# RemoteSensingTools/vSmartMOM.jl

Hardware: AMD Instinct MI355X
Metric: spectral-points/s (whole node) for rt_run, O2-A band (higher is better)
Workload: dtype f64; 1 GPU; C2: O2-A 759-770 nm, nStokes=3, Nquad=20 (N=60), 40 layers, 10000 spectral points/GPU, m=0..2, Rayleigh+synthetic O2 absorption, Lambertian 0.15; ranks=1, collective_backend=none (1 rank), N=60, layers=40, points_per_gpu=10000, fourier_moments=3

## Files before the change

include/vsmartmom_hip.h:

```cpp
#ifndef VSMARTMOM_HIP_H
#define VSMARTMOM_HIP_H

#include <stddef.h>
#include <stdint.h>

#ifdef __cplusplus
extern "C" {
#endif

typedef enum vsm_status {
  VSM_OK = 0,
  VSM_ERR_INVALID_ARG = 1,
  VSM_ERR_UNSUPPORTED = 2,
  VSM_ERR_HIP = 3,
  VSM_ERR_NO_DEVICE = 4
} vsm_status;

typedef enum vsm_iface {
  VSM_IFACE_00 = 0,
  VSM_IFACE_01 = 1,
  VSM_IFACE_10 = 2,
  VSM_IFACE_11 = 3
} vsm_iface;

// ... 387 lines not shown
int vsm_run_create_view_f64(const vsm_quad_f64* q, int S, int nm, const int* m_h, const int* coupling_h, void* workspace,
                            size_t workspace_bytes, unsigned flags, int nrows, const int* rows_h, vsm_run** run);
int vsm_run_create_view_f32(const vsm_quad_f32* q, int S, int nm, const int* m_h, const int* coupling_h, void* workspace,
                            size_t workspace_bytes, unsigned flags, int nrows, const int* rows_h, vsm_run** run);
int vsm_run_layer_f64(vsm_run* run, int ndoubl, const double* dtau, const double* varpi, const double* tau_sum,
                      const double* F0, int ncomp, const double* const* Zpp, const double* const* Zmp, long long z_stride,
                      const double* fcomp, int toa, const int* layer_coupling_h, void* stream);
int vsm_run_layer_f32(vsm_run* run, int ndoubl, const float* dtau, const float* varpi, const float* tau_sum,
                      const float* F0, int ncomp, const float* const* Zpp, const float* const* Zmp, long long z_stride,
                      const float* fcomp, int toa, const int* layer_coupling_h, void* stream);
int vsm_run_export_f64(vsm_run* run, const vsm_composite_f64* comps, void* stream);
int vsm_run_export_f32(vsm_run* run, const vsm_composite_f32* comps, void* stream);
int vsm_run_import_f64(vsm_run* run, const vsm_composite_f64* comps, void* stream);
int vsm_run_import_f32(vsm_run* run, const vsm_composite_f32* comps, void* stream);
int vsm_run_zw_tail(vsm_run* run);
int vsm_run_view_rows(vsm_run* run, int nrows, const int* rows_h);
int vsm_run_view_block(const vsm_run* run, int block, int* im, int* n, int* nv, int* local_rows);
int vsm_run_view_rows(vsm_run* run, int nrows, const int* rows_h);
int vsm_run_view_block(const vsm_run* run, int block, int* im, int* n, int* nv, int* local_rows);
int vsm_run_destroy(vsm_run* run);
enum { VSM_SURFACE_LAMBERTIAN_SCALAR = 0, VSM_SURFACE_LAMBERTIAN_SPECTRAL = 1, VSM_SURFACE_BRDF = 2 };
enum { VSM_SURFACE_LAYER_IDENTITY = 1 };
unsigned vsm_surface_layer_flags(int kind, int m, int has_surface_source);
int vsm_run_export_moment_f64(vsm_run* run, int im, const vsm_composite_f64* comp, void* stream);
int vsm_run_export_moment_f32(vsm_run* run, int im, const vsm_composite_f32* comp, void* stream);
int vsm_run_export_sources_f64(vsm_run* run, int im, const vsm_composite_f64* comp, void* stream);
int vsm_run_export_sources_f32(vsm_run* run, int im, const vsm_composite_f32* comp, void* stream);
int vsm_run_surface_f64(vsm_run* run, int im, int iface, const vsm_added_f64* added_surface, int identity, int matrices,
                        const vsm_composite_f64* comp, double* work, void* stream);
int vsm_run_surface_f32(vsm_run* run, int im, int iface, const vsm_added_f32* added_surface, int identity, int matrices,
                        const vsm_composite_f32* comp, float* work, void* stream);
int vsm_run_guard_once(vsm_run* run);
int vsm_run_counters(const vsm_run* run, int* counts_h);
int vsm_stokes_coupling_f64(int N, int n_stokes, int nblocks, const double* Zpp, const double* Zmp, int* mask_d, void* stream);
int vsm_stokes_coupling_f32(int N, int n_stokes, int nblocks, const float* Zpp, const float* Zmp, int* mask_d, void* stream);

typedef struct vsm_added_rs_f64 {
  double *ier_mp, *iet_pp, *ier_pm, *iet_mm;
  double *ieJ0_p, *ieJ0_m;
  int K;
  int reserved;
} vsm_added_rs_f64;
typedef struct vsm_added_rs_f32 {
  float *ier_mp, *iet_pp, *ier_pm, *iet_mm;
  float *ieJ0_p, *ieJ0_m;
  int K;
  int reserved;
} vsm_added_rs_f32;
typedef struct vsm_composite_rs_f64 {
  double *ieR_mp, *ieR_pm, *ieT_pp, *ieT_mm;
  double *ieJ0_p, *ieJ0_m;
  int K;
  int reserved;
} vsm_composite_rs_f64;
typedef struct vsm_composite_rs_f32 {
  float *ieR_mp, *ieR_pm, *ieT_pp, *ieT_mm;
  float *ieJ0_p, *ieJ0_m;
  int K;
  int reserved;
} vsm_composite_rs_f32;
typedef struct vsm_rrs_f64 {
  const int* shift;
  const double* varpi_ie;
  const double* fscatt;
  const double* Zpp;
  const double* Zmp;
// ... 306 lines not shown
```

vsmartmom.jl_amd/_lib.py:

```python
from __future__ import annotations

import ctypes as C
import os

_HERE = os.path.dirname(os.path.abspath(__file__))
LIB_PATH = os.environ.get("VSM_LIB_PATH") or os.path.join(_HERE, "lib", "libvsmartmom_hip.so")


class VSMError(RuntimeError):
    pass


class vsm_quad_f64(C.Structure):
    _fields_ = [("mu", C.c_void_p), ("wt", C.c_void_p), ("N", C.c_int), ("n_stokes", C.c_int),
                ("i_mu0", C.c_int), ("mu0", C.c_double)]


class vsm_quad_f32(C.Structure):
    _fields_ = [("mu", C.c_void_p), ("wt", C.c_void_p), ("N", C.c_int), ("n_stokes", C.c_int),
                ("i_mu0", C.c_int), ("mu0", C.c_float)]


class vsm_added(C.Structure):
    _fields_ = [("r_mp", C.c_void_p), ("t_pp", C.c_void_p), ("r_pm", C.c_void_p), ("t_mm", C.c_void_p),
# ... 115 lines not shown
    "vsm_interaction_inelastic_rrs_{T}": (_I, [_I, _I, _I, _P, _P, _P, _P, _P, _P, _P]),
    "vsm_copy_added_to_composite_ie_{T}": (_I, [_I, _I, _P, _P, _P]),
    "vsm_postprocess_vza_ie_{T}": (_I, [_I, _I, _I, _I, _I, _P, _P, _P, _P, _P, _P, _P]),
    "vsm_ss_column_{T}": (_I, [_P, _I, _I, _I, _P, _P, _P, _P, _P, _P, _P, _P, _P, _P, _I, _P, _P, _P, _P, _P, _P, _P]),
    "vsm_ss_column_lin_{T}": (_I, [_P, _I, _I, _I, _I, _I, _I, _I, _I, _P, _P, _P, _P, _P, _P, _P, _P, _P, _P, _I, _P, _P, _P, _P, _P, _P, _P,
                                   _P, _P, _I, _P, _P, _P, _P, _P]),
    "vsm_ss_column_rrs_{T}": (_I, [_P, _I, _I, _I, _I, _P, _P, _P, _P, _P, _P, _P, _P, _I, _I, _P, _P, _P, _P, _P]),
    "vsm_ss_column_rrs_lin_{T}": (_I, [_P, _I, _I, _I, _I, _I, _I, _I, _I, _P, _P, _P, _P, _P, _P, _P, _P, _P, _P, _P, _I, _I, _P, _P, _P,
                                       _P, _P]),
    "vsm_exact_ss_path1_{T}": (_I, [_I, _I, _I, _I, _I, _P, _P, _P, _P, "{R}", _P, _P, _P]),
    "vsm_exact_ss_path2_{T}": (_I, [_I, _I, _I, _I, _I, _P, _P, _I, _P, "{R}", _P, _P, _P]),
    "vsm_exact_ss_path34_{T}": (_I, [_I, _I, _I, _I, _I, _P, _P, _P, _P, _P, _P, _P, _P, "{R}", _P, _P, _P, _P]),
    "vsm_exact_ss_jac12_{T}": (_I, [_I, _I, _I, _I, _I, _P, _P, _P, _P, _I, _P, "{R}", _P, _P, _P, _P, _P, _P, _P]),
    "vsm_run_supported": (_I, [_I, _I, _I]),
    "vsm_run_workspace_bytes": (_SZ, [_I, _I, _I, _I, _P]),
    "vsm_run_supported_f32": (_I, [_I, _I, _I]),
    "vsm_run_workspace_bytes_f32": (_SZ, [_I, _I, _I, _I, _P]),
    "vsm_run_create_{T}": (_I, [_P, _I, _I, _P, _P, _P, _SZ, _P]),
    "vsm_run_create_ex_{T}": (_I, [_P, _I, _I, _P, _P, _P, _SZ, C.c_uint, _P]),
    "vsm_run_create_view_{T}": (_I, [_P, _I, _I, _P, _P, _P, _SZ, C.c_uint, _I, _P, _P]),
    "vsm_run_layer_{T}": (_I, [_P, _I, _P, _P, _P, _P, _I, _P, _P, _LL, _P, _I, _P, _P]),
    "vsm_run_export_{T}": (_I, [_P, _P, _P]),
    "vsm_run_import_{T}": (_I, [_P, _P, _P]),
    "vsm_run_zw_tail": (_I, [_P]),
    "vsm_run_view_rows": (_I, [_P, _I, _P]),
    "vsm_run_view_block": (_I, [_P, _I, _P, _P, _P, _P]),
    "vsm_run_destroy": (_I, [_P]),
    "vsm_surface_layer_flags": (C.c_uint, [_I, _I, _I]),
    "vsm_run_export_moment_{T}": (_I, [_P, _I, _P, _P]),
    "vsm_run_export_sources_{T}": (_I, [_P, _I, _P, _P]),
    "vsm_run_surface_{T}": (_I, [_P, _I, _I, _P, _I, _I, _P, _P, _P]),
    "vsm_run_guard_once": (_I, [_P]),
    "vsm_run_counters": (_I, [_P, _P]),
    "vsm_stokes_coupling_{T}": (_I, [_I, _I, _I, _P, _P, _P, _P]),
    "vsm_level_radiance_work_elems": (_SZ, [_I, _I]),
    "vsm_level_radiance_{T}": (_I, [_I, _I, _I, _I, _P, _P, _P, _P, _P, _LL, _P, _P, _P, _P, _P, _P, _P]),
    "vsm_level_radiance_oplevel_{T}": (_I, [_I, _I, _I, _I, _P, _P, _P, _P, _P, _LL, _P, _P, _P, _P, _P, _P, _P]),
    "vsm_level_radiance_src_{T}": (_I, [_I, _I, _I, _I, _P, _P, _P, _I, _P, _P, _LL, _P, _P, _P, _P, _P, _P, _P]),
    "vsm_level_flux_{T}": (_I, [_I, _I, _I, _P, _I, _P, _P, _LL, _P, _I, _P, _P, "{R}", _P, _P, _P, _P]),
    "vsm_surface_emission_response_{T}": (_I, [_I, _I, _I, _I, _P, _I, _P, _P, _P, _P, _P, _LL, _P, _P, _P]),
    "vsm_level_radiance_ie_{T}": (_I, [_I, _I, _I, _I, _P, _I, _P, _P, _P, _P, _LL, _P, _P, _P, _P, _P, _P, _P, _P, _P, _P, _P]),
    "vsm_level_flux_ie_{T}": (_I, [_I, _I, _I, _I, _P, _P, _P, _LL, _P, _P, _P, _P, _P, _P, _I, _P, _P, "{R}", _P, _P, _P, _P]),
    "vsm_level_radiance_lin_{T}": (_I, [_I, _I, _I, _I, _I, _I, _P, _P, _P, _P, _LL, _P, _P, _P, _LL, _P, _P, _LL, _LL, _P, _P, _P, _P, _P,
                                        _P]),
    "vsm_level_radiance_lin_src_{T}": (_I, [_I, _I, _I, _I, _I, _I, _I, _P, _P, _P, _P, _LL, _P, _P, _P, _LL, _P, _P, _LL, _LL, _P, _P, _P,
                                            _P, _P, _P, _P, _P]),
    "vsm_level_flux_lin_{T}": (_I, [_I, _I, _I, _I, _I, _I, _P, _P, _LL, _P, _P, _P, _LL, _P, _P, _LL, _LL, _P, _P, _P, _I, _P, _P,
                                    "{R}", _P, _P, _P, _I, _P, _P]),
    "vsm_mie_work_elems": (_SZ, [_I, _I, _I]),
    "vsm_mie_nai2": (_I, [_I, _I, _I, C.c_double, C.c_double, C.c_double, _P, _P, _P, _P, _P, _P, _P, _P, _P, _P, _P]),
    "vsm_mie_lin_work_elems": (_SZ, [_I, _I, _I]),
    "vsm_mie_nai2_lin": (_I, [_I, _I, _I, C.c_double, C.c_double, C.c_double] + [_P] * 16),
    "vsm_dbge_work_elems": (_SZ, [_I, _I]),
    "vsm_truncate_dbge": (_I, [_I, _I, _I, C.c_double, _P, _P, _P, _P, _P, _P, _P, _P, _P, _P]),
    "vsm_dbge_lin_work_elems": (_SZ, [_I, _I]),
    "vsm_truncate_dbge_lin": (_I, [_I, _I, _I, C.c_double] + [_P] * 15),
    "vsm_absorption_chunk": (_I, []),
    "vsm_absorption_work_elems": (_SZ, [_I, _I]),
    "vsm_absorption_xsec": (_I, [_I, _I, _I, _I] + [_P] * 15 + [C.c_double, C.c_double, _I, _I, _I, _P, _P, _P]),
    "vsm_absorption_lin_chunk": (_I, []),
    "vsm_absorption_lin_work_elems": (_SZ, [_I, _I]),
    "vsm_absorption_xsec_lin": (_I, [_I, _I, _I, _I] + [_P] * 16 + [C.c_double, C.c_double, _I, _I, _I] + [_P] * 6),
    "vsm_absorption_profile_slots": (_I, [_I, _I, _I] + [_P] * 6),
    "vsm_absorption_lut_chunk": (_I, []),
    "vsm_absorption_lut_span": (_I, []),
    "vsm_absorption_lut_work_elems": (_SZ, [_I, _I, _I, _I]),
# ... 107 lines not shown
```

vsmartmom.jl_amd/core_rt.py:

```python
from __future__ import annotations

import contextlib
import ctypes as C
import dataclasses
import math
import os
import warnings
from dataclasses import dataclass
from typing import List, Optional

import numpy as np
import torch

from . import _lib
from . import host_model as H
from .architectures import GPU, CPU, architecture, array_type, devi, synchronize_if_gpu, to_host

IFACE = {"00": 0, "01": 1, "10": 2, "11": 3}
MOMENT_BATCH = 4
MOMENT_BATCH_MAX = 24
MOMENT_BATCHING = True
THERMAL_FUSION = True
NATIVE_RUN = True
NATIVE_SOURCES_ONLY = True
NATIVE_VIEW_ROWS = True
VIEW_ROWS_MAX = 16
NATIVE_ZW_TAIL = True
NATIVE_IDENTITY_SURFACE = True
NATIVE_DROPIN = True
REFERENCE_ORDER = False


def _require_gpu(arch):
    if not isinstance(arch, GPU):
        raise _lib.VSMError("vsmartmom.jl_amd provides the MI355X path only; architecture %r has no compute path here "
                            "(no CPU fallback by design)" % (arch,))
    if not torch.cuda.is_available():
        raise _lib.VSMError("no MI355X visible to HIP (torch.cuda.is_available() is False)")
    if arch.device_index != torch.cuda.current_device():
        raise _lib.VSMError("architecture GPU(%d) is not the current HIP device (%d): one process per GPU -- call "
                            "torch.cuda.set_device(%d) first" % (arch.device_index, torch.cuda.current_device(),
                                                                 arch.device_index))


def _torch_dtype(FT):
    return torch.float64 if np.dtype(FT) == np.float64 else torch.float32


def _stream_ptr():
    return C.c_void_p(torch.cuda.current_stream().cuda_stream)


def _ptr(t: Optional[torch.Tensor]):
    return C.c_void_p(0 if t is None else t.data_ptr())


def to_device_matrix(A: np.ndarray, arch, FT) -> torch.Tensor:
    A = np.asarray(A, dtype=FT)
    if A.ndim == 2:
        A = A[None]
    return array_type(arch)(np.ascontiguousarray(A.transpose(0, 2, 1)))
# ... 1020 lines not shown
                               work=self.work, keep_added=keep_added)
            if iz + 1 in tops_at:
                for k, comp in zip(rest, comps_l):
                    keep_top(k, iz + 1, comp.snapshot_top())

    def _native_moments(self):
        if not NATIVE_RUN or getattr(self, "coupling", None) is None or not self.moments:
            return set()
        eps2 = 2 * np.finfo(self.FT).eps
        for iz, ly in enumerate(self.moments[0]["layers"]):
            p = ly["props"]
            if p.max_tau_varpi <= eps2 or (iz > 0 and ly["iface"] != "11") or (p.fcomp is not None and p.fcomp.shape[1] > 4):
                return set()
        return {i for i, mom in enumerate(self.moments) if run_supported(self.dt, self.N, self.pol.n, int(self.coupling[mom["m"]]))}

    def _run_layers_native(self, group, comps, sources_only: bool = True, export_at=None, view_rows=None, keep_native: bool = False):
        L = _lib.lib()
        self._drop_lazy()
        nm, N, S, ns = len(group), self.N, self.S, self.pol.n
        marr = (C.c_int * nm)(*[int(mom["m"]) for mom in group])
        carr = (C.c_int * nm)(*[int(self.coupling[mom["m"]]) for mom in group])
        nbytes = run_workspace_bytes(self.dt, N, ns, S, nm, carr)
        ws = getattr(self, "_native_ws", None)
        if ws is None or ws.numel() * 8 < nbytes:
            ws = self._native_ws = _lib.poison(torch.empty(max(nbytes // 8, 2), dtype=torch.float64, device=self.dev))
        q = self.dq.cstruct()
        run = C.c_void_p()
        run_create_(self.dt, q, S, nm, marr, carr, ws, nbytes, sources_only, view_rows, run)
        ref = RunRef(run, self.__dict__.setdefault("_run_counts", {}), keep=(ws, self.dq))
        try:
            _lib.check(L.vsm_run_guard_once(run))
            if NATIVE_ZW_TAIL and not torch.cuda.is_current_stream_capturing():
                _lib.check(L.vsm_run_zw_tail(run))
            for iz in range(self.Nz):
                ly0 = group[0]["layers"][iz]
                props = [mom["layers"][iz]["props"] for mom in group]
                p0 = props[0]
                zpp = (C.c_void_p * nm)(*[p.Zpp.data_ptr() for p in props])
                zmp = (C.c_void_p * nm)(*[p.Zmp.data_ptr() for p in props])
                ncomp = 0 if p0.fcomp is None else int(p0.fcomp.shape[1])
                lc = (C.c_int * nm)(*[self._layer_coupling(mom["m"], iz) for mom in group])
                run_layer_native_(run, nm, int(ly0["nd"]), ly0["dtau"], p0.varpi, ly0["tau_sum"], self.F0, ncomp, zpp, zmp,
                                  0 if ncomp else p0.z_stride, p0.fcomp, iz == 0, lc, self.dt)
                if export_at and (iz + 1) in export_at:
                    cc = (type(comps[0].cstruct()) * nm)(*[c.cstruct() for c in comps])
                    _lib.call("vsm_run_export", self.dt, run, cc, _stream_ptr())
                    export_at[iz + 1](comps)
            if keep_native:
                for im, (mom, c) in enumerate(zip(group, comps)):
                    c.drop_native()
                    mask = int(self.coupling[mom["m"]])
                    c._native = NativeSlot(run, int(mom["m"]), mask, stokes_groups(ns, mask), ref, im)
                    ref.refs += 1
            else:
                cc = (type(comps[0].cstruct()) * nm)(*[c.cstruct() for c in comps])
                _lib.call("vsm_run_export", self.dt, run, cc, _stream_ptr())
        finally:
            ref.release()

    def thermal_slot(self) -> "ThermalSlot":
        if self._thermal is None:
            self._thermal = ThermalSlot(self)
        return self._thermal

    def _thermal_slot(self, mom, weight):
        th = self.thermal_slot()
# ... 175 lines not shown
```

vsmartmom.jl_amd/csrc/vsm_elemental.h:

```cpp
#pragma once
#include "vsm_common.h"

namespace vsm {

template <typename T>
__device__ __forceinline__ T expm1_small(T y) {
  T q = T(1.0 / 39916800.0);
  q = fma(q, y, T(1.0 / 3628800.0));
  q = fma(q, y, T(1.0 / 362880.0));
  q = fma(q, y, T(1.0 / 40320.0));
  q = fma(q, y, T(1.0 / 5040.0));
  q = fma(q, y, T(1.0 / 720.0));
  q = fma(q, y, T(1.0 / 120.0));
  q = fma(q, y, T(1.0 / 24.0));
  q = fma(q, y, T(1.0 / 6.0));
  q = fma(q, y, T(0.5));
  q = fma(q, y, T(1.0));
  return q * y;
}
template <typename T>
__device__ __forceinline__ T expdiff_tab_thin(T xi, T xj, T ai, T aj, T ej) {
  const T dlt = xi - xj;
  return (fabs(dlt) > T(0.125) * fmax(xi, xj)) ? (ai - aj) : ej * expm1_small<T>(-dlt);
}
template <typename T>
__device__ __forceinline__ T expdiff_tab_thick(T xi, T xj, T ei, T ej) {
  const T dlt = xi - xj;
  const T v = ((dlt < T(0)) ? ei : ej) * (-expm1(-fabs(dlt)));
  return (dlt < T(0)) ? v : -v;
}

__device__ __forceinline__ double geo_div(double a, double b) { return a / b; }
__device__ __forceinline__ float geo_div(float a, float b) { return __fdividef(a, b); }

template <typename T>
__device__ __forceinline__ void elemental_pair(T w, T zp, T zm, T mi, T xi, T ai, T ei, T mj, T xj, T aj, T ej, T wct, bool diag,
                                               bool thick, T& rr, T& tt) {
  rr = w * zm * geo_div(mj, mi + mj) * wct * (-(ai + aj + ai * aj));
  T ediff;
  if (thick) ediff = expdiff_tab_thick<T>(xi, xj, ei, ej); else ediff = expdiff_tab_thin<T>(xi, xj, ai, aj, ej);
  const T t_off = w * zp * geo_div(mj, mi - mj) * wct * ediff;
  const T t_1 = w * zp * xi * wct;
  const T t_same = diag ? ei * (T(1) + t_1) : ej * t_1;
  tt = (mi == mj) ? t_same : t_off;
}

}
```

vsmartmom.jl_amd/csrc/vsm_native.hip:

```cpp
#include <stdlib.h>

#include <vector>

#include "vsm_native_dev.h"
#include "vsm_native_run.h"

#ifndef VSM_NATIVE_PARK_RT
#define VSM_NATIVE_PARK_RT 3
#endif

namespace vsm {

struct nlayer_comps {
  double* c[NSUB_MAX];
};

namespace {

template <int RT, int KS, int KZ = KS, bool TILE = false>
__device__ __forceinline__ void ned_body(nsmem<RT, (4 * KS + 2 > 16 * RT)>& sm, npos<RT>& p, int n, int gsz, unsigned uvmask, int ndoubl,
                                         const double* __restrict__ img, nstrip<RT>& r_s, nstrip<RT>& t_s, int* status) {
  using G = ngeo<RT>;
  constexpr unsigned dP = 0, dQ = G::AF * 8;
  double* jp = sm.vec[0];
// ... 1153 lines not shown
    }
    R[naf_idx<RT>(i, j)] = rv;
    T[naf_idx<RT>(i, j)] = tv;
  }
  if (ph == 0) {
    const int i0 = ns * q.i_mu0;
    const double mu0n = q.mu[i0];
    const double x0 = d / mu0n, e0 = exp(-x0), a0 = expm1(-x0);
    double zp = 0.0, zm = 0.0;
    for (int qq = 0; qq < ns; ++qq) {
      const long long zo = fi + (long long)N * (i0 + qq);
      const double f = F0[qq + (long long)ns * s];
      zp += zget(Zp, zo) * f;
      zm += zget(Zm, zo) * f;
    }
    double rr, tt;
    elemental_pair(w, zp, zm, mi, xi, ai, ei, mu0n, x0, a0, e0, (m == 0) ? 0.5 : 0.25, false, thick || x0 >= 0.5, rr, tt);
    const double att = exp(-tau_sum[s] / mu0n);
    const double vp = (i < n) ? tt * att : 0.0;
    const double vm = (i < n) ? rr * att * sg : 0.0;
    const double expk0 = exp(-d / q.mu0);
    out[2 * G::AF + i] = vp;
    out[2 * G::AF + NP + i] = vm;
    out[2 * G::AF + 2 * NP + i] = expk0;
    if (riders_in) {
      T[naf_idx<RT>(i, c1)] = vp;
      T[naf_idx<RT>(i, c2)] = vm * expk0;
      R[naf_idx<RT>(i, c1)] = vm;
      R[naf_idx<RT>(i, c2)] = vp;
    }
  }
}

template <typename T>
struct ngroup_map {
  int ngroups;
  int grp_of[4];
  int pos_in[4];
  int gsz[4];
  int rt[4];
  int n[4];
  T* base[4];
};
__device__ __forceinline__ int nat_idx_rt(const double*, int rt, int i, int j) {
  const int w = j >> 4, l15 = j & 15, ta = i >> 4, mm = i & 15, kq = mm & 3, r = mm >> 2;
  const int lane = (kq << 4) | l15, u = 2 * ta + (r >> 1);
  return ((w * 2 * rt + u) * 64 + lane) * 2 + (r & 1);
}
__device__ __forceinline__ int nat_idx_rt(const float*, int rt, int i, int j) {
  const int w = j >> 4, l15 = j & 15, ta = i >> 4, mm = i & 15, kq = mm & 3, r = mm >> 2;
  return ((w * rt + ta) * 64 + ((kq << 4) | l15)) * 4 + r;
}
__device__ __forceinline__ void nat_elem_rt(const double*, int rt, int e, int& i, int& j) {
  const int half = e & 1, lane = (e >> 1) & 63, unit = (e >> 7) % (2 * rt), w = (e >> 7) / (2 * rt);
  i = 16 * (unit >> 1) + (lane >> 4) + 4 * (2 * (unit & 1) + half), j = 16 * w + (lane & 15);
}
__device__ __forceinline__ void nat_elem_rt(const float*, int rt, int e, int& i, int& j) {
  const int r = e & 3, lane = (e >> 2) & 63, ta = (e >> 8) % rt, w = (e >> 8) / rt;
  i = 16 * ta + (lane >> 4) + 4 * r, j = 16 * w + (lane & 15);
}
template <typename T>
__global__ __launch_bounds__(256) void k_native_export(int N, int ns, int src, int view, ngroup_map<T> gm, nview vw, composite<T> c) {
  const int s = blockIdx.x, tid = threadIdx.x;
  const long long NN = (long long)N * N;
  T* out[4] = {c.R_mp + s * NN, c.R_pm + s * NN, c.T_pp + s * NN, c.T_mm + s * NN};
  for (int e = tid; e < N * N; e += 256) {
// ... 293 lines not shown
  }
#undef VSM_NI
  return VSM_ERR_UNSUPPORTED;
}
namespace {

template <int RT>
static void launch_pre(bool mix, const quad<double>& q, int S, int nsub, int n, int ndoubl, const double* dtau, const double* varpi,
                       const double* tau_sum, const double* F0, const npre_args<double>& a, double* pre, hipStream_t st) {
  const dim3 grid(S, nsub), block(64 * RT);
  if (mix)
    hipLaunchKernelGGL((k_elemental_native<RT, true>), grid, block, 0, st, q, n, ndoubl, dtau, varpi, tau_sum, F0, a, pre);
  else
    hipLaunchKernelGGL((k_elemental_native<RT, false>), grid, block, 0, st, q, n, ndoubl, dtau, varpi, tau_sum, F0, a, pre);
}

static void native_launch_pre(int rt, bool mix, const quad<double>& q, int S, int nsub, int n, int ndoubl, const double* dtau,
                              const double* varpi, const double* tau_sum, const double* F0, const npre_args<double>& a, double* pre,
                              hipStream_t st) {
  switch (rt) {
    case 1: launch_pre<1>(mix, q, S, nsub, n, ndoubl, dtau, varpi, tau_sum, F0, a, pre, st); break;
    case 2: launch_pre<2>(mix, q, S, nsub, n, ndoubl, dtau, varpi, tau_sum, F0, a, pre, st); break;
    case 3: launch_pre<3>(mix, q, S, nsub, n, ndoubl, dtau, varpi, tau_sum, F0, a, pre, st); break;
    case 4: launch_pre<4>(mix, q, S, nsub, n, ndoubl, dtau, varpi, tau_sum, F0, a, pre, st); break;
    case 5: launch_pre<5>(mix, q, S, nsub, n, ndoubl, dtau, varpi, tau_sum, F0, a, pre, st); break;
    default: launch_pre<6>(mix, q, S, nsub, n, ndoubl, dtau, varpi, tau_sum, F0, a, pre, st); break;
  }
}
static void native_launch_pre(int rt, bool mix, const quad<float>& q, int S, int nsub, int n, int ndoubl, const float* dtau,
                              const float* varpi, const float* tau_sum, const float* F0, const npre_args<float>& a, float* pre,
                              hipStream_t st) {
  native32_launch_pre(rt, mix, q, S, nsub, n, ndoubl, dtau, varpi, tau_sum, F0, a, pre, st);
}
static int native_launch_layer(const nat_sub& h, int S, int nsub, int ndoubl, int toa, int src, const double* pre, double* const* comps,
                               int* status, const nview* vw, hipStream_t st) {
  return launch_layer_native(h.ks, h.ks - h.kz, S, nsub, h.n, h.uvmask, h.gsz, ndoubl, toa, src, pre, comps, status, vw, st);
}
static int native_launch_layer(const nat_sub& h, int S, int nsub, int ndoubl, int toa, int, const float* pre, float* const* comps,
                               int* status, const nview*, hipStream_t st) {
  return native32_launch_layer(h.ks, S, nsub, h.n, h.uvmask, h.gsz, ndoubl, toa, pre, comps, status, st);
}

template <typename T>
static ngroup_map<T> group_map(const vsm_run* run, int im) {
  ngroup_map<T> gm;
  gm.ngroups = 0;
  for (int a = 0; a < 4; ++a) {
    gm.grp_of[a] = gm.pos_in[a] = 0;
    gm.gsz[a] = gm.rt[a] = 1;
    gm.n[a] = 0;
    gm.base[a] = nullptr;
  }
  for (const nat_sub& sb : run->subs) {
    if (sb.im != im) continue;
    const int g = gm.ngroups++;
    gm.gsz[g] = sb.gsz;
    gm.rt[g] = sb.rt;
    gm.n[g] = sb.n;
    gm.base[g] = static_cast<T*>(run->ws) + sb.comp_off;
    for (int k = 0; k < sb.gsz; ++k) {
      gm.grp_of[sb.g[k]] = g;
      gm.pos_in[sb.g[k]] = k;
    }
  }
  return gm;
}
// ... 151 lines not shown
    return true;
  };
  if (!run->guard_once || run->layers == 1) {
    nguard_args<T> ga;
    for (int k = 0; k < NSUB_MAX; ++k) {
      const int im = k < run->nm ? k : 0;
      VSM_REQUIRE(Zpp[im] && Zmp[im], "vsm_run_layer: null Z of moment %d", im);
      ga.zp[k] = Zpp[im];
      ga.zm[k] = Zmp[im];
      ga.allowed[k] = 0;
    }
    for (const nat_sub& sb : run->subs) {
      if (trivial(sb)) continue;
      for (int a = 0; a < sb.gsz; ++a)
        for (int b = 0; b < sb.gsz; ++b) ga.allowed[sb.im] |= 1u << (4 * sb.g[a] + sb.g[b]);
    }
    const int nmat = ncomp ? ncomp : (z_stride ? run->S : 1);
    hipLaunchKernelGGL((k_coupling_guard<T>), dim3(nmat, run->nm), dim3(256), 0, st, run->N, run->ns,
                       ncomp ? (long long)run->N * run->N : z_stride, ga, status);
    VSM_LAUNCH_CHECK("k_coupling_guard");
    ++run->guards;
  }
  T* const ws = static_cast<T*>(run->ws);
  const int src = (run->flags & VSM_RUN_SOURCES_ONLY) ? 1 : 0;
  const int view = (run->flags & VSM_RUN_VIEW_ROWS) ? 1 : 0;
  size_t pre_total = 0;
  for (const nat_sub& sb : run->subs)
    if (!trivial(sb)) pre_total += pre_stride_rt(sb.rt) * (size_t)run->S;
  T* pre = nullptr;
  if (pre_total) {
    pre = static_cast<T*>(scratch(pre_total * sizeof(T), 3, st));
    if (!pre) return VSM_ERR_HIP;
  }
  size_t off = 0;
  for (const auto& cl : run->classes) {
    const nat_sub& h = run->subs[cl[0]];
    std::vector<int> act, triv[3];
    for (int i : cl) {
      if (!trivial(run->subs[i])) {
        act.push_back(i);
        run->pure_diag[i] = 0;
      } else if (toa) {
        triv[1].push_back(i);
        run->pure_diag[i] = 1;
      } else {
        triv[run->pure_diag[i] ? 2 : 0].push_back(i);
      }
    }
    for (int mode = 0; mode < 3; ++mode) {
      if (triv[mode].empty()) continue;
      ndiag_args<T> da;
      const int nt = (int)triv[mode].size();
      for (int k = 0; k < NSUB_MAX; ++k) {
        const nat_sub& sb = run->subs[triv[mode][k < nt ? k : 0]];
        da.comp[k] = ws + sb.comp_off;
        da.gsz[k] = sb.gsz;
        da.g0[k] = sb.g[0] | (sb.g[1] << 4) | (sb.g[2] << 8) | (sb.g[3] << 12);
      }
      hipLaunchKernelGGL((k_native_diag_layer<T>), dim3(run->S, nt), dim3(256), 0, st, q, h.rt, h.n, (T)ldexp(1.0, ndoubl), mode,
                         src, view, dtau, da, view ? view_of(run, triv[mode]) : nview{});
      VSM_LAUNCH_CHECK("k_native_diag_layer");
    }
    const int nsub = (int)act.size();
    if (!nsub) continue;
    npre_args<T> pa;
    T* lc[NSUB_MAX];
    for (int k = 0; k < NSUB_MAX; ++k) {
      const nat_sub& sb = run->subs[act[k < nsub ? k : 0]];
      pa.s[k].m = sb.m;
      pa.s[k].gsz = sb.gsz;
      for (int a = 0; a < 4; ++a) pa.s[k].g[a] = sb.g[a];
      VSM_REQUIRE(Zpp[sb.im] && Zmp[sb.im], "vsm_run_layer: null Z of moment %d", sb.im);
      pa.s[k].z = zsrc<T>{Zpp[sb.im], Zmp[sb.im], ncomp ? 0 : z_stride, ncomp, fcomp};
      lc[k] = ws + sb.comp_off;
    }
    T* pre_cl = pre + off;
    off += pre_stride_rt(h.rt) * (size_t)run->S * nsub;
    native_launch_pre(h.rt, ncomp > 0, q, run->S, nsub, h.n, ndoubl, dtau, varpi, tau_sum, F0, pa, pre_cl, st);
    VSM_LAUNCH_CHECK("k_elemental_native");
    const nview vw = view ? view_of(run, act) : nview{};
    const int rc = native_launch_layer(h, run->S, nsub, ndoubl, toa, src, pre_cl, lc, status, view ? &vw : nullptr, st);
    if (rc) return rc;
  }
  return VSM_OK;
}

template <typename T, typename CS, bool IMPORT>
static int run_convert(vsm_run* run, const CS* comps, void* stream) {
  VSM_REQUIRE(run && comps, "vsm_run_export / import: null argument");
  VSM_REQUIRE(run->elem_size == (int)sizeof(T), "vsm_run_export / import: the run was created for %d-byte arrays", run->elem_size);
  if (IMPORT) ++run->imports;
  if (run->S == 0) return VSM_OK;
  if (IMPORT) {
    run->pure_diag.assign(run->subs.size(), 0);
    run->flags &= ~(unsigned)VSM_RUN_ZW_TAIL;
    for (nat_sub& sb : run->subs) sb.kz = sb.ks;
    run->guard_once = false;
  }
  for (int im = 0; im < run->nm; ++im) {
    const CS& c = comps[im];
    VSM_REQUIRE(c.R_mp && c.R_pm && c.T_pp && c.T_mm && c.J0_p && c.J0_m, "vsm_run_export / import: null composite array (moment %d)", im);
    const composite<T> cc{c.R_mp, c.R_pm, c.T_pp, c.T_mm, c.J0_p, c.J0_m};
    const ngroup_map<T> gm = group_map<T>(run, im);
    const int view = (run->flags & VSM_RUN_VIEW_ROWS) ? 1 : 0;
    const nview vw = view ? view_of_moment(run, im) : nview{};
    if (IMPORT)
      hipLaunchKernelGGL((k_native_import<T>), dim3(run->S), dim3(256), 0, as_stream(stream), run->N, run->ns, view, gm, vw, cc);
    else
      hipLaunchKernelGGL((k_native_export<T>), dim3(run->S), dim3(256), 0, as_stream(stream), run->N, run->ns,
                         (run->flags & VSM_RUN_SOURCES_ONLY) ? 1 : 0, view, gm, vw, cc);
    VSM_LAUNCH_CHECK("k_native_export / import");
    if (!IMPORT) ++run->exports_full;
// ... 164 lines not shown
int vsm_run_import_f32(vsm_run* run, const vsm_composite_f32* comps, void* stream) {
  return run_convert<float, vsm_composite_f32, true>(run, comps, stream);
}

int vsm_run_export_moment_f64(vsm_run* run, int im, const vsm_composite_f64* comp, void* stream) {
  return run_export_moment<double>(run, im, comp, true, stream, "vsm_run_export_moment");
}
int vsm_run_export_moment_f32(vsm_run* run, int im, const vsm_composite_f32* comp, void* stream) {
  return run_export_moment<float>(run, im, comp, true, stream, "vsm_run_export_moment");
}
int vsm_run_export_sources_f64(vsm_run* run, int im, const vsm_composite_f64* comp, void* stream) {
  return run_export_moment<double>(run, im, comp, false, stream, "vsm_run_export_sources");
}
int vsm_run_export_sources_f32(vsm_run* run, int im, const vsm_composite_f32* comp, void* stream) {
  return run_export_moment<float>(run, im, comp, false, stream, "vsm_run_export_sources");
}

int vsm_run_surface_f64(vsm_run* run, int im, int iface, const vsm_added_f64* added_surface, int identity, int matrices,
                        const vsm_composite_f64* comp, double* work, void* stream) {
  return run_surface<double>(run, im, iface, added_surface, identity, matrices, comp, work, stream, vsm_interaction_f64);
}
int vsm_run_surface_f32(vsm_run* run, int im, int iface, const vsm_added_f32* added_surface, int identity, int matrices,
                        const vsm_composite_f32* comp, float* work, void* stream) {
  return run_surface<float>(run, im, iface, added_surface, identity, matrices, comp, work, stream, vsm_interaction_f32);
}

int vsm_run_guard_once(vsm_run* run) {
  VSM_REQUIRE(run, "vsm_run_guard_once: null argument");
  VSM_REQUIRE(run->layers == 0 && run->imports == 0, "vsm_run_guard_once: the run has taken layer steps or an import already");
  run->guard_once = true;
  return VSM_OK;
}

int vsm_run_counters(const vsm_run* run, int* counts) {
  VSM_REQUIRE(run && counts, "vsm_run_counters: null argument");
  counts[0] = run->exports_full;
  counts[1] = run->exports_src;
  counts[2] = run->surface_ia;
  counts[3] = run->guards;
  return VSM_OK;
}

int vsm_stokes_coupling_f64(int N, int n_stokes, int nblocks, const double* Zpp, const double* Zmp, int* mask_d, void* stream) {
  return stokes_coupling<double>(N, n_stokes, nblocks, Zpp, Zmp, mask_d, stream);
}
int vsm_stokes_coupling_f32(int N, int n_stokes, int nblocks, const float* Zpp, const float* Zmp, int* mask_d, void* stream) {
  return stokes_coupling<float>(N, n_stokes, nblocks, Zpp, Zmp, mask_d, stream);
}

}

#endif
```

vsmartmom.jl_amd/csrc/vsm_native_run.h:

```cpp
#pragma once
#include <vector>

#include "vsm_internal.h"

namespace vsm {

constexpr int NSUB_MAX = VSM_MM_MAX;

struct nat_sub {
  int im;
  int m;
  int gsz, g[4];
  unsigned uvmask;
  int n, rt, ks;
  int kz;
  size_t comp_off;
  int nv;
  int vrow[VSM_RUN_VIEW_MAX];
};

struct nview {
  int nv[NSUB_MAX];
  unsigned pk[NSUB_MAX][VSM_RUN_VIEW_MAX / 4];
  __host__ __device__ int row(int k, int v) const { return (int)((pk[k][v >> 2] >> (8 * (v & 3))) & 255u); }
  __host__ __device__ int find(int k, int r) const {
    int at = -1;
    for (int v = 0; v < nv[k]; ++v) at = row(k, v) == r ? v : at;
    return at;
  }
};

}

struct vsm_run {
  const void *mu, *wt;
  int N, ns, i_mu0;
  double mu0;
  int elem_size;
  int S, nm;
  unsigned flags;
  std::vector<int> view_rows;
  std::vector<int> m;
  std::vector<vsm::nat_sub> subs;
  std::vector<std::vector<int>> classes;
  void* ws;
  size_t ws_elems;
  int layers = 0;
  int imports = 0;
  std::vector<char> pure_diag;
  bool guard_once = false;
  int exports_full = 0, exports_src = 0, surface_ia = 0, guards = 0;
};

namespace vsm {

constexpr int NATIVE_MAX_ROWS = 96;
constexpr int NATIVE32_MAX_ROWS = 128;

constexpr int rt_of(int n) {
  const int ks = (n + 3) / 4;
  return (ks % 4 == 0 && ks >= 4) ? ks / 4 : (4 * ks + 2 + 15) / 16;
}
constexpr size_t comp_stride_rt(int rt) { return (size_t)4 * (16 * rt) * (16 * rt) + 2 * 16 * rt; }
constexpr size_t pre_stride_rt(int rt) { return (size_t)2 * (16 * rt) * (16 * rt) + 3 * 16 * rt; }

template <typename T>
struct nsub_pre {
  int m, gsz;
  int g[4];
  zsrc<T> z;
};
template <typename T>
struct npre_args {
  nsub_pre<T> s[NSUB_MAX];
};

void native32_launch_pre(int rt, bool mix, const quad<float>& q, int S, int nsub, int n, int ndoubl, const float* dtau,
                         const float* varpi, const float* tau_sum, const float* F0, const npre_args<float>& a, float* pre,
                         hipStream_t st);
int native32_launch_layer(int ks, int S, int nsub, int n, unsigned uvmask, int gsz, int ndoubl, int toa, const float* pre,
                          float* const* comps, int* status, hipStream_t st);

}
```

Before: 27000 spectral-points/s.

## Fuse per-class elemental prepass into one shared kernel reusing per-node pair factors

Adds a single f64 elemental prepass kernel that handles every non-trivial sub-block of all Fourier/Stokes classes in one launch per layer. It computes the geometry and exponential pair factors once per quadrature node pair in LDS and shares them across sub-blocks, instead of recomputing them in a separate launch per class. It is enabled from Python only when mu and weights are identical across the Stokes components of each node. This is meant to cut redundant exp/expm1 and division work and launch overhead. In exchange it adds a large argument struct, heavier LDS use and a host memcpy check at setup.

```diff
diff --git a/include/vsmartmom_hip.h b/include/vsmartmom_hip.h
--- a/include/vsmartmom_hip.h
+++ b/include/vsmartmom_hip.h
@@ -443,6 +443,7 @@
                         const vsm_composite_f32* comp, float* work, void* stream);
 int vsm_run_guard_once(vsm_run* run);
 int vsm_run_counters(const vsm_run* run, int* counts_h);
+int vsm_run_shared_prepass(vsm_run* run, int on, int* active);
 int vsm_stokes_coupling_f64(int N, int n_stokes, int nblocks, const double* Zpp, const double* Zmp, int* mask_d, void* stream);
 int vsm_stokes_coupling_f32(int N, int n_stokes, int nblocks, const float* Zpp, const float* Zmp, int* mask_d, void* stream);
 
diff --git a/vsmartmom.jl_amd/_lib.py b/vsmartmom.jl_amd/_lib.py
--- a/vsmartmom.jl_amd/_lib.py
+++ b/vsmartmom.jl_amd/_lib.py
@@ -171,6 +171,7 @@
     "vsm_run_surface_{T}": (_I, [_P, _I, _I, _P, _I, _I, _P, _P, _P]),
     "vsm_run_guard_once": (_I, [_P]),
     "vsm_run_counters": (_I, [_P, _P]),
+    "vsm_run_shared_prepass": (_I, [_P, _I, _P]),
     "vsm_stokes_coupling_{T}": (_I, [_I, _I, _I, _P, _P, _P, _P]),
     "vsm_level_radiance_work_elems": (_SZ, [_I, _I]),
     "vsm_level_radiance_{T}": (_I, [_I, _I, _I, _I, _P, _P, _P, _P, _P, _LL, _P, _P, _P, _P, _P, _P, _P]),
diff --git a/vsmartmom.jl_amd/core_rt.py b/vsmartmom.jl_amd/core_rt.py
--- a/vsmartmom.jl_amd/core_rt.py
+++ b/vsmartmom.jl_amd/core_rt.py
@@ -27,6 +27,7 @@
 VIEW_ROWS_MAX = 16
 NATIVE_ZW_TAIL = True
 NATIVE_IDENTITY_SURFACE = True
+NATIVE_SHARED_PREPASS = True
 NATIVE_DROPIN = True
 REFERENCE_ORDER = False
 
@@ -1113,6 +1114,8 @@
             _lib.check(L.vsm_run_guard_once(run))
             if NATIVE_ZW_TAIL and not torch.cuda.is_current_stream_capturing():
                 _lib.check(L.vsm_run_zw_tail(run))
+            if NATIVE_SHARED_PREPASS and hasattr(L, "vsm_run_shared_prepass") and not torch.cuda.is_current_stream_capturing():
+                _lib.check(L.vsm_run_shared_prepass(run, 1, None))
             for iz in range(self.Nz):
                 ly0 = group[0]["layers"][iz]
                 props = [mom["layers"][iz]["props"] for mom in group]
diff --git a/vsmartmom.jl_amd/csrc/vsm_elemental.h b/vsmartmom.jl_amd/csrc/vsm_elemental.h
--- a/vsmartmom.jl_amd/csrc/vsm_elemental.h
+++ b/vsmartmom.jl_amd/csrc/vsm_elemental.h
@@ -45,4 +45,27 @@
   tt = (mi == mj) ? t_same : t_off;
 }
 
+template <typename T>
+struct pair_factors {
+  T g_r, e_r, g_t, ediff;
+};
+template <typename T>
+__device__ __forceinline__ pair_factors<T> elemental_factors(T mi, T xi, T ai, T ei, T mj, T xj, T aj, T ej, bool thick) {
+  pair_factors<T> f;
+  f.g_r = geo_div(mj, mi + mj);
+  f.e_r = -(ai + aj + ai * aj);
+  if (thick) f.ediff = expdiff_tab_thick<T>(xi, xj, ei, ej); else f.ediff = expdiff_tab_thin<T>(xi, xj, ai, aj, ej);
+  f.g_t = geo_div(mj, mi - mj);
+  return f;
 }
+template <typename T>
+__device__ __forceinline__ void elemental_apply(T w, T zp, T zm, const pair_factors<T>& f, T xi, T ei, T ej, T wct, bool diag, bool same,
+                                                T& rr, T& tt) {
+  rr = w * zm * f.g_r * wct * f.e_r;
+  const T t_off = w * zp * f.g_t * wct * f.ediff;
+  const T t_1 = w * zp * xi * wct;
+  const T t_same = diag ? ei * (T(1) + t_1) : ej * t_1;
+  tt = same ? t_same : t_off;
+}
+
+}
diff --git a/vsmartmom.jl_amd/csrc/vsm_native.hip b/vsmartmom.jl_amd/csrc/vsm_native.hip
--- a/vsmartmom.jl_amd/csrc/vsm_native.hip
+++ b/vsmartmom.jl_amd/csrc/vsm_native.hip
@@ -1209,6 +1209,209 @@
   }
 }
 
+__host__ __device__ __forceinline__ int nall_even(int v) { return (v + 1) & ~1; }
+static size_t nall_lds_bytes(int nq, int vtot) {
+  return sizeof(double) * (size_t)(4 * nq * (nq | 1) + 4 * nq + 5 * nall_even(nq) + 2 * vtot) + sizeof(unsigned) * (size_t)nq;
+}
+constexpr int NALL_U = 4;
+__device__ __forceinline__ int nall_node(int r, int gsz) {
+  return gsz == 1 ? r : (gsz == 2 ? (r >> 1) : (gsz == 3 ? (int)(((unsigned)r * 43691u) >> 17) : (r >> 2)));
+}
+template <bool MIX>
+__global__ __launch_bounds__(256) void k_elemental_native_all(quad<double> q, int nsub, int vtot, int ndoubl,
+                                                              const double* __restrict__ dtau, const double* __restrict__ varpi,
+                                                              const double* __restrict__ tau_sum, const double* __restrict__ F0,
+                                                              long long zs, int ncomp_in, const double* __restrict__ fcomp,
+                                                              nall_args<double> a, double* __restrict__ pre) {
+  extern __shared__ nd2_t nall_lds[];
+  __shared__ int thick_flag;
+  const int s = blockIdx.x, tid = threadIdx.x;
+  const int N = q.N, ns = q.n_stokes, nq = N / ns, nqp = nq | 1, nqe = nall_even(nq);
+  double* pairs = reinterpret_cast<double*>(nall_lds);
+  double* srcf = pairs + 4 * nq * nqp;
+  double* mus = srcf + 4 * nq;
+  double* xs = mus + nqe;
+  double* es = xs + nqe;
+  double* ems = es + nqe;
+  double* wts = ems + nqe;
+  double* svp = wts + nqe;
+  double* svm = svp + vtot;
+  unsigned* same = reinterpret_cast<unsigned*>(svm + vtot);
+  const double d = dtau[s], w = varpi[s];
+  const int ncomp = MIX ? ncomp_in : 0;
+  const long long NNz = (long long)N * N;
+  const long long zbase = ncomp ? 0 : (long long)s * zs;
+  double fk[4] = {0.0, 0.0, 0.0, 0.0};
+#pragma unroll
+  for (int k = 0; k < 4; ++k)
+    if (k < ncomp) fk[k] = fcomp[(long long)s * ncomp + k];
+  auto zget = [&](const double* Z, long long zo) {
+    if (ncomp == 0) return Z[zo];
+    double acc = 0.0;
+#pragma unroll
+    for (int k = 0; k < 4; ++k)
+      if (k < ncomp) acc += fk[k] * Z[k * NNz + zo];
+    return acc;
+  };
+  if (tid < nq) {
+    const double mu = q.mu[tid * ns];
+    const double x = d / mu;
+    mus[tid] = mu;
+    xs[tid] = x;
+    es[tid] = exp(-x);
+    ems[tid] = expm1(-x);
+    wts[tid] = q.wt[tid * ns];
+  }
+  if (tid == 0) thick_flag = 0;
+  __syncthreads();
+  if (tid < nq && xs[tid] >= 0.5) thick_flag = 1;
+  __syncthreads();
+  const bool thick = thick_flag != 0;
+  const int i0 = ns * q.i_mu0;
+  const double mu0n = q.mu[i0];
+  const double x0 = d / mu0n, e0 = exp(-x0), a0 = expm1(-x0);
+  for (int p = tid; p < nq * nq; p += 256) {
+    const int na = p / nq, nb = p - na * nq;
+    const pair_factors<double> f = elemental_factors<double>(mus[na], xs[na], ems[na], es[na], mus[nb], xs[nb], ems[nb], es[nb], thick);
+    double* o = pairs + 4 * (na * nqp + nb);
+    o[0] = f.g_r;
+    o[1] = f.e_r;
+    o[2] = f.g_t;
+    o[3] = f.ediff;
+  }
+  if (tid < nq) {
+    const double mi = mus[tid];
+    unsigned bits = 0u;
+    for (int nb = 0; nb < nq; ++nb) bits |= (mi == mus[nb]) ? (1u << nb) : 0u;
+    same[tid] = bits;
+    const pair_factors<double> f =
+        elemental_factors<double>(mi, xs[tid], ems[tid], es[tid], mu0n, x0, a0, e0, thick || x0 >= 0.5);
+    double* o = srcf + 4 * tid;
+    o[0] = f.g_r;
+    o[1] = f.e_r;
+    o[2] = f.g_t;
+    o[3] = f.ediff;
+  }
+  __syncthreads();
+  const double expk0 = exp(-d / q.mu0);
+  for (int idx = tid; idx < vtot; idx += 256) {
+    int k = 0;
+    while (k + 1 < nsub && idx >= a.s[k + 1].voff) ++k;
+    const nsub_all<double>& sp = a.s[k];
+    const int i = idx - sp.voff, NP = 16 * sp.rt, AF = NP * NP;
+    double vp = 0.0, vm = 0.0;
+    if (i < sp.n) {
+      const int na = nall_node(i, sp.gsz), ci = (sp.gpk >> (4 * (i - na * sp.gsz))) & 15;
+      const int fi = na * ns + ci;
+      const double* Zp = sp.Zpp + zbase;
+      const double* Zm = sp.Zmp + zbase;
+      double zp = 0.0, zm = 0.0;
+      for (int qq = 0; qq < ns; ++qq) {
+        const long long zo = fi + (long long)N * (i0 + qq);
+        const double f = F0[qq + (long long)ns * s];
+        zp += zget(Zp, zo) * f;
+        zm += zget(Zm, zo) * f;
+      }
+      pair_factors<double> f;
+      f.g_r = srcf[4 * na];
+      f.e_r = srcf[4 * na + 1];
+      f.g_t = srcf[4 * na + 2];
+      f.ediff = srcf[4 * na + 3];
+      double rr, tt;
+      elemental_apply<double>(w, zp, zm, f, xs[na], es[na], e0, (sp.m == 0) ? 0.5 : 0.25, false, mus[na] == mu0n, rr, tt);
+      const double att = exp(-tau_sum[s] / mu0n);
+      const double sg = (ndoubl >= 1 && ci >= 2) ? -1.0 : 1.0;
+      vp = tt * att;
+      vm = rr * att * sg;
+    }
+    svp[idx] = vp;
+    svm[idx] = vm;
+    double* out = pre + sp.off + (long long)s * (2 * AF + 3 * NP);
+    out[2 * AF + i] = vp;
+    out[2 * AF + NP + i] = vm;
+    out[2 * AF + 2 * NP + i] = expk0;
+  }
+  __syncthreads();
+  const int lane = tid & 63, kk = lane >> 4, l15 = lane & 15;
+  const int wave = __builtin_amdgcn_readfirstlane(tid >> 6);
+  for (int k = 0; k < nsub; ++k) {
+    const nsub_all<double>& sp = a.s[k];
+    const int rt = sp.rt, n = sp.n, gsz = sp.gsz, gpk = sp.gpk, NP = 16 * rt, AF = NP * NP;
+    const bool m0 = sp.m == 0;
+    const double* Zp = sp.Zpp + zbase;
+    const double* Zm = sp.Zmp + zbase;
+    double* R = pre + sp.off + (long long)s * (2 * AF + 3 * NP);
+    double* T = R + AF;
+    const int Kend = ((n + 3) >> 2) << 2;
+    const int c1 = Kend, c2 = Kend + 1;
+    const bool riders_in = ndoubl > 0 && c2 < NP;
+    const double* bvp = svp + sp.voff;
+    const double* bvm = svm + sp.voff;
+    int t = wave, ks = 0;
+    while (t >= rt) {
+      t -= rt;
+      ++ks;
+    }
+    while (ks < 4 * rt) {
+      int bt[NALL_U], bks[NALL_U], bi[NALL_U], bj[NALL_U], bna[NALL_U], bnb[NALL_U], bci[NALL_U];
+      double zp[NALL_U], zm[NALL_U];
+#pragma unroll
+      for (int u = 0; u < NALL_U; ++u) {
+        bt[u] = t;
+        bks[u] = ks;
+        const int kc = min(ks, 4 * rt - 1);
+        const int i = 16 * t + (l15 ^ (kk | ((kc & 3) << 2))), j = 4 * kc + kk;
+        const int ic = min(i, n - 1), jc = min(j, n - 1);
+        const int na = nall_node(ic, gsz), ci = (gpk >> (4 * (ic - na * gsz))) & 15;
+        const int nb = nall_node(jc, gsz), cj = (gpk >> (4 * (jc - nb * gsz))) & 15;
+        const long long zo = (na * ns + ci) + (long long)N * (nb * ns + cj);
+        zp[u] = zget(Zp, zo);
+        zm[u] = zget(Zm, zo);
+        bi[u] = i;
+        bj[u] = j;
+        bna[u] = na;
+        bnb[u] = nb;
+        bci[u] = ci;
+        t += 4;
+        while (t >= rt) {
+          t -= rt;
+          ++ks;
+        }
+      }
+#pragma unroll
+      for (int u = 0; u < NALL_U; ++u) {
+        if (bks[u] >= 4 * rt) break;
+        const int i = bi[u], j = bj[u], na = bna[u], nb = bnb[u];
+        const nd2_t* fp = reinterpret_cast<const nd2_t*>(pairs + 4 * (na * nqp + nb));
+        const nd2_t f01 = fp[0], f23 = fp[1];
+        pair_factors<double> f;
+        f.g_r = f01.x;
+        f.e_r = f01.y;
+        f.g_t = f23.x;
+        f.ediff = f23.y;
+        const double wt = wts[nb];
+        const double wct = m0 ? wt / 2.0 : wt / 4.0;
+        const double ei = es[na];
+        double rr, tt;
+        elemental_apply<double>(w, zp[u], zm[u], f, xs[na], ei, es[nb], wct, i == j, ((same[na] >> nb) & 1u) != 0u, rr, tt);
+        const bool active = wct > num<double>::eps();
+        const double sg = (ndoubl >= 1 && bci[u] >= 2) ? -1.0 : 1.0;
+        const bool in = i < n && j < n;
+        double rv = in ? (active ? rr * sg : 0.0) : 0.0;
+        double tv = in ? (active ? tt : ((i == j) ? ei : 0.0)) : 0.0;
+        if (riders_in && (j == c1 || j == c2)) {
+          const double vp = bvp[i], vm = bvm[i];
+          tv = (j == c1) ? vp : vm * expk0;
+          rv = (j == c1) ? vm : vp;
+        }
+        const int o = (bks[u] * rt + bt[u]) * 64 + lane;
+        R[o] = rv;
+        T[o] = tv;
+      }
+    }
+  }
+}
+
 template <typename T>
 struct ngroup_map {
   int ngroups;
@@ -1568,6 +1771,30 @@
                               hipStream_t st) {
   native32_launch_pre(rt, mix, q, S, nsub, n, ndoubl, dtau, varpi, tau_sum, F0, a, pre, st);
 }
+static void native_launch_pre_all(bool mix, const quad<double>& q, int S, int ndoubl, const double* dtau, const double* varpi,
+                                  const double* tau_sum, const double* F0, long long zs, int ncomp, const double* fcomp,
+                                  const std::vector<nsub_all<double>>& blocks, double* pre, hipStream_t st) {
+  const int nq = q.N / q.n_stokes;
+  for (size_t b0 = 0; b0 < blocks.size(); b0 += NALL_MAX) {
+    const int nsub = (int)std::min(blocks.size() - b0, (size_t)NALL_MAX);
+    nall_args<double> a;
+    int vtot = 0;
+    for (int k = 0; k < NALL_MAX; ++k) {
+      a.s[k] = blocks[b0 + (k < nsub ? k : 0)];
+      a.s[k].voff = vtot;
+      if (k < nsub) vtot += 16 * a.s[k].rt;
+    }
+    const size_t lds = nall_lds_bytes(nq, vtot);
+    if (mix)
+      hipLaunchKernelGGL((k_elemental_native_all<true>), dim3(S), dim3(256), lds, st, q, nsub, vtot, ndoubl, dtau, varpi, tau_sum, F0, zs,
+                         ncomp, fcomp, a, pre);
+    else
+      hipLaunchKernelGGL((k_elemental_native_all<false>), dim3(S), dim3(256), lds, st, q, nsub, vtot, ndoubl, dtau, varpi, tau_sum, F0,
+                         zs, ncomp, fcomp, a, pre);
+  }
+}
+static void native_launch_pre_all(bool, const quad<float>&, int, int, const float*, const float*, const float*, const float*, long long,
+                                  int, const float*, const std::vector<nsub_all<float>>&, float*, hipStream_t) {}
 static int native_launch_layer(const nat_sub& h, int S, int nsub, int ndoubl, int toa, int src, const double* pre, double* const* comps,
                                int* status, const nview* vw, hipStream_t st) {
   return launch_layer_native(h.ks, h.ks - h.kz, S, nsub, h.n, h.uvmask, h.gsz, ndoubl, toa, src, pre, comps, status, vw, st);
@@ -1785,6 +2012,34 @@
     pre = static_cast<T*>(scratch(pre_total * sizeof(T), 3, st));
     if (!pre) return VSM_ERR_HIP;
   }
+  const bool shared = run->shared_pre && sizeof(T) == 8;
+  if (shared && pre_total) {
+    std::vector<nsub_all<T>> blocks;
+    size_t off_cl = 0;
+    for (const auto& cl : run->classes) {
+      int k = 0;
+      for (int i : cl) {
+        const nat_sub& sb = run->subs[i];
+        if (trivial(sb)) continue;
+        VSM_REQUIRE(Zpp[sb.im] && Zmp[sb.im], "vsm_run_layer: null Z of moment %d", sb.im);
+        nsub_all<T> b;
+        b.Zpp = Zpp[sb.im];
+        b.Zmp = Zmp[sb.im];
+        b.off = (long long)(off_cl + pre_stride_rt(sb.rt) * (size_t)run->S * k);
+        b.m = sb.m;
+        b.gsz = sb.gsz;
+        b.gpk = sb.g[0] | (sb.g[1] << 4) | (sb.g[2] << 8) | (sb.g[3] << 12);
+        b.n = sb.n;
+        b.rt = sb.rt;
+        b.voff = 0;
+        blocks.push_back(b);
+        ++k;
+      }
+      off_cl += pre_stride_rt(run->subs[cl[0]].rt) * (size_t)run->S * k;
+    }
+    native_launch_pre_all(ncomp > 0, q, run->S, ndoubl, dtau, varpi, tau_sum, F0, ncomp ? 0 : z_stride, ncomp, fcomp, blocks, pre, st);
+    VSM_LAUNCH_CHECK("k_elemental_native_all");
+  }
   size_t off = 0;
   for (const auto& cl : run->classes) {
     const nat_sub& h = run->subs[cl[0]];
@@ -1829,8 +2084,10 @@
     }
     T* pre_cl = pre + off;
     off += pre_stride_rt(h.rt) * (size_t)run->S * nsub;
-    native_launch_pre(h.rt, ncomp > 0, q, run->S, nsub, h.n, ndoubl, dtau, varpi, tau_sum, F0, pa, pre_cl, st);
-    VSM_LAUNCH_CHECK("k_elemental_native");
+    if (!shared) {
+      native_launch_pre(h.rt, ncomp > 0, q, run->S, nsub, h.n, ndoubl, dtau, varpi, tau_sum, F0, pa, pre_cl, st);
+      VSM_LAUNCH_CHECK("k_elemental_native");
+    }
     const nview vw = view ? view_of(run, act) : nview{};
     const int rc = native_launch_layer(h, run->S, nsub, ndoubl, toa, src, pre_cl, lc, status, view ? &vw : nullptr, st);
     if (rc) return rc;
@@ -2061,6 +2318,24 @@
   return VSM_OK;
 }
 
+int vsm_run_shared_prepass(vsm_run* run, int on, int* active) {
+  VSM_REQUIRE(run, "vsm_run_shared_prepass: null argument");
+  VSM_REQUIRE(run->layers == 0, "vsm_run_shared_prepass: the run has taken layer steps already");
+  run->shared_pre = false;
+  if (active) *active = 0;
+  if (!on || run->elem_size != 8 || run->S == 0) return VSM_OK;
+  const int N = run->N, ns = run->ns, nq = N / ns;
+  if (nq > NALL_NODES_MAX) return VSM_OK;
+  std::vector<double> mw(2 * (size_t)N);
+  VSM_HIP(hipMemcpy(mw.data(), run->mu, sizeof(double) * (size_t)N, hipMemcpyDefault));
+  VSM_HIP(hipMemcpy(mw.data() + N, run->wt, sizeof(double) * (size_t)N, hipMemcpyDefault));
+  for (int i = 0; i < N; ++i)
+    if (mw[i] != mw[(i / ns) * ns] || mw[N + i] != mw[N + (i / ns) * ns]) return VSM_OK;
+  run->shared_pre = true;
+  if (active) *active = 1;
+  return VSM_OK;
+}
+
 int vsm_run_counters(const vsm_run* run, int* counts) {
   VSM_REQUIRE(run && counts, "vsm_run_counters: null argument");
   counts[0] = run->exports_full;
diff --git a/vsmartmom.jl_amd/csrc/vsm_native_run.h b/vsmartmom.jl_amd/csrc/vsm_native_run.h
--- a/vsmartmom.jl_amd/csrc/vsm_native_run.h
+++ b/vsmartmom.jl_amd/csrc/vsm_native_run.h
@@ -49,6 +49,7 @@
   int imports = 0;
   std::vector<char> pure_diag;
   bool guard_once = false;
+  bool shared_pre = false;
   int exports_full = 0, exports_src = 0, surface_ia = 0, guards = 0;
 };
 
@@ -75,6 +76,21 @@
   nsub_pre<T> s[NSUB_MAX];
 };
 
+constexpr int NALL_MAX = 16;
+constexpr int NALL_NODES_MAX = 32;
+template <typename T>
+struct nsub_all {
+  const T *Zpp, *Zmp;
+  long long off;
+  int m, gsz, gpk;
+  int n, rt;
+  int voff;
+};
+template <typename T>
+struct nall_args {
+  nsub_all<T> s[NALL_MAX];
+};
+
 void native32_launch_pre(int rt, bool mix, const quad<float>& q, int S, int nsub, int n, int ndoubl, const float* dtau,
                          const float* varpi, const float* tau_sum, const float* F0, const npre_args<float>& a, float* pre,
                          hipStream_t st);
```

After: 27080 spectral-points/s (median of 6 runs). About the same (+0.3%).
